# liusongxiang/efficient_tts

Hardware: AMD Instinct MI355X
Metric: mel-frames/sec (EFTS-CNN forward, batch 64/GPU, 80-mel LJSpeech shape) (higher is better)
Workload: dtype bf16; 1 GPU; EFTS-CNN forward (teacher-forced, no_grad) B=64 phon=128 mel=800 80-bin; batch_per_gpu=64, phoneme_len=128, mel_len=800, precision=bf16, parallelism=replicas x1

## Files before the change

### efficient_tts_amd/csrc/efts_prenet.hip

```cpp
#include <hip/hip_runtime.h>
#include <stdint.h>

#include "efts_rowsweep.h"

namespace efts {

struct FlArgs {
    const float* x;
    const char* w;
    const float* bias;
    float* y_f32;
    char* y;
    char* y_lo;
    long ldw, ldo, ldy;
    int B, T, Tp, cin, n;
    int act;
    float slope;
    int y_split;
};

constexpr int FL_NCB = 4;

template <int SPLIT, int KS>
__global__ __launch_bounds__(512, 2) void frame_linear_kernel(FlArgs p) {
    extern __shared__ __attribute__((aligned(16))) char smem[];
    constexpr int WF_BYTES = KS * FL_NCB * SPLIT * 1024;
    const int tid = threadIdx.x, lane = tid & 63, wave = tid >> 6, lrow = lane & 31, lhalf = lane >> 5;
    const int ncq = p.n / (32 * FL_NCB);
    const int ns = (p.cin + 15) >> 4;
    for (int unit = blockIdx.x; unit < p.B * ncq; unit += gridDim.x) {
    const int b = unit / ncq, cq = unit - b * ncq;
    const int c0 = cq * 32 * FL_NCB;
    if (unit != (int)blockIdx.x) __syncthreads();

    for (int idx = tid; idx < ns * FL_NCB * 64; idx += 512) {
        const int l = idx & 63, cb = (idx >> 6) % FL_NCB, s = idx / (64 * FL_NCB);
        const int k0 = 16 * s + 8 * (l >> 5);
        const char* src = p.w + (long)(c0 + cb * 32 + (l & 31)) * p.ldw + (SPLIT == 1 ? k0 * 2 : (k0 >> 5) * 128 + (k0 & 31) * 2);
        char* d = smem + ((s * FL_NCB + cb) * SPLIT) * 1024 + l * 16;
        *(u32x4*)d = *(const u32x4*)src;
        if constexpr (SPLIT == 2) *(u32x4*)(d + 1024) = *(const u32x4*)(src + 64);
    }
    float bv[FL_NCB];
#pragma unroll
    for (int cb = 0; cb < FL_NCB; ++cb) bv[cb] = p.bias ? p.bias[c0 + cb * 32 + lrow] : 0.f;
    __syncthreads();

    char* const st = smem + WF_BYTES + wave * 8192;
    const RowOut o{p.y_f32, p.y, p.y_lo, p.ldo, p.ldy, p.y_split};
    const int nrb = (p.T + 31) >> 5;
    for (int rb = wave; rb < nrb; rb += 8) {
        const int t = rb * 32 + lrow;
        const bool live = t < p.T;
        const float* xr = p.x + ((long)b * p.T + (live ? t : 0)) * p.cin;
        bf16x8 ah[KS], al[SPLIT == 2 ? KS : 1];
        (void)al;
#pragma unroll
        for (int s = 0; s < KS; ++s) {
            const int k0 = s * 16 + lhalf * 8;
            float f[8];
#pragma unroll
            for (int u = 0; u < 8; ++u) f[u] = 0.f;
            if (live && s < ns && k0 + 8 <= p.cin) {
                const float4 q0 = *(const float4*)(xr + k0), q1 = *(const float4*)(xr + k0 + 4);
                f[0] = q0.x; f[1] = q0.y; f[2] = q0.z; f[3] = q0.w; f[4] = q1.x; f[5] = q1.y; f[6] = q1.z; f[7] = q1.w;
            }
            u32x4 h4, l4;
            split8(f, &h4, &l4);
            ah[s] = __builtin_bit_cast(bf16x8, h4);
            if constexpr (SPLIT == 2) al[s] = __builtin_bit_cast(bf16x8, l4);
        }
        f32x16 acc[FL_NCB];
#pragma unroll
        for (int cb = 0; cb < FL_NCB; ++cb)
#pragma unroll
            for (int r = 0; r < 16; ++r) acc[cb][r] = 0.f;
#pragma unroll
        for (int s = 0; s < KS; ++s) {
            if (s < ns) {
                bf16x8 bh[FL_NCB], bl[SPLIT == 2 ? FL_NCB : 1];
                (void)bl;
#pragma unroll
                for (int cb = 0; cb < FL_NCB; ++cb) {
                    const char* src = smem + ((s * FL_NCB + cb) * SPLIT) * 1024 + lane * 16;
                    bh[cb] = *(const bf16x8*)src;
                    if constexpr (SPLIT == 2) bl[cb] = *(const bf16x8*)(src + 1024);
                }
                if constexpr (SPLIT == 2) {
#pragma unroll
                    for (int cb = 0; cb < FL_NCB; ++cb) acc[cb] = __builtin_amdgcn_mfma_f32_32x32x16_bf16(al[s], bh[cb], acc[cb], 0, 0, 0);
#pragma unroll
                    for (int cb = 0; cb < FL_NCB; ++cb) acc[cb] = __builtin_amdgcn_mfma_f32_32x32x16_bf16(ah[s], bl[cb], acc[cb], 0, 0, 0);
                }
#pragma unroll
                for (int cb = 0; cb < FL_NCB; ++cb) acc[cb] = __builtin_amdgcn_mfma_f32_32x32x16_bf16(ah[s], bh[cb], acc[cb], 0, 0, 0);
            }
        }
#pragma unroll
        for (int hp = 0; hp < FL_NCB / 2; ++hp)
            sweep64<true>(acc[2 * hp], acc[2 * hp + 1], st, lane, o, (long)b * p.Tp + rb * 32, p.T - rb * 32, c0 + hp * 64, bv[2 * hp], bv[2 * hp + 1],
                          p.act, p.slope);
    }
    }
}

}

using namespace efts;

extern "C" int efts_frame_linear(const efts_frame_linear_args* a, void* stream) {
    if (!a) return efts_fail(EFTS_EINVAL, "efts_frame_linear: null args");
    if (!a->x || !a->w || (!a->y && !a->y_f32)) return efts_fail(EFTS_EINVAL, "efts_frame_linear: null operand / no output");
    if (!(a->split == 1 || a->split == 2) || (a->y && !(a->y_split == 1 || a->y_split == 2))) return efts_fail(EFTS_EINVAL, "efts_frame_linear: split / y_split must be 1 or 2");
    if (a->B <= 0 || a->T <= 0 || a->Tp < a->T || a->cin <= 0 || a->cin > 128 || (a->cin & 7) || a->n <= 0 || a->n % (32 * FL_NCB))
        return efts_fail(EFTS_ESHAPE, "efts_frame_linear: cin must be a multiple of 8 up to 128, n a multiple of 128, T <= Tp");
    const int kch = a->split == 1 ? 64 : 32, nchunk = (a->cin + kch - 1) / kch;
    if (a->ldw < (int64_t)nchunk * 128 || (a->ldw & 15) || ((uintptr_t)a->w & 15) || ((uintptr_t)a->x & 15) || ((a->cin * 4) & 15))
        return efts_fail(EFTS_EALIGN, "efts_frame_linear: weight plane stride / alignment, frames must be 16-byte aligned rows");
    if ((a->y && ((a->ldy & 15) || ((uintptr_t)a->y & 15) || ((uintptr_t)a->y_lo & 15))) || (a->y_f32 && ((a->ldo & 3) || ((uintptr_t)a->y_f32 & 15))))
        return efts_fail(EFTS_EALIGN, "efts_frame_linear: output rows must be 16-byte aligned");
    if (a->y_split == 2 && a->y_lo) return efts_fail(EFTS_EINVAL, "efts_frame_linear: y_lo is for split-1 output planes");
    FlArgs k;
    k.x = a->x; k.w = (const char*)a->w; k.bias = a->bias; k.y_f32 = a->y_f32; k.y = (char*)a->y; k.y_lo = (char*)a->y_lo;
    k.ldw = a->ldw; k.ldo = a->ldo; k.ldy = a->ldy; k.B = a->B; k.T = a->T; k.Tp = a->Tp; k.cin = a->cin; k.n = a->n;
    k.act = a->act; k.slope = a->slope; k.y_split = a->y ? a->y_split : 0;
    int wgs = a->B * (a->n / (32 * FL_NCB));
    if (a->max_workgroups > 0 && a->max_workgroups < wgs) wgs = a->max_workgroups;
    const dim3 grid((unsigned)wgs);
#define EFTS_FL(S, N)                                                                                                                \
    do {                                                                                                                             \
        static bool attr = false;                                                                                                    \
        if (!attr) { (void)hipFuncSetAttribute((const void*)frame_linear_kernel<S, N>, hipFuncAttributeMaxDynamicSharedMemorySize, 160 * 1024); attr = true; } \
        hipLaunchKernelGGL((frame_linear_kernel<S, N>), grid, dim3(512), (size_t)N * FL_NCB * S * 1024 + 8 * 8192, (hipStream_t)stream, k);  \
    } while (0)
    const bool small = a->cin <= 80;
    if (a->split == 1) { if (small) EFTS_FL(1, 5); else EFTS_FL(1, 8); }
    else { if (small) EFTS_FL(2, 5); else EFTS_FL(2, 8); }
#undef EFTS_FL
    return efts_check_launch("efts_frame_linear");
}
```

### efficient_tts_amd/csrc/efts_rowsweep.h

```cpp
#pragma once
#include "efts_mma.h"

namespace efts {

struct RowOut {
    float* y_f32;
    char* y;
    char* y_lo;
    long ldo, ldy;
    int y_split;
};

__device__ __forceinline__ void gstore_b128(void* p, u32x4 v) {
    *(u32x4*)p = v;
    asm volatile("s_nop 4" ::"v"(v));
}

__device__ __forceinline__ void split8(const float* f, u32x4* hi, u32x4* lo) {
    float r[8], d0, d1;
    *hi = u32x4{pack_bf16x2(f[0], f[1], &r[0], &r[1]), pack_bf16x2(f[2], f[3], &r[2], &r[3]),
                pack_bf16x2(f[4], f[5], &r[4], &r[5]), pack_bf16x2(f[6], f[7], &r[6], &r[7])};
    *lo = u32x4{pack_bf16x2(r[0], r[1], &d0, &d1), pack_bf16x2(r[2], r[3], &d0, &d1),
                pack_bf16x2(r[4], r[5], &d0, &d1), pack_bf16x2(r[6], r[7], &d0, &d1)};
}

template <bool EPI>
__device__ __forceinline__ void sweep64(const f32x16& a0, const f32x16& a1, char* st, int lane, const RowOut& o, long orow0,
                                        int rows_live, int col0, float b0, float b1, int act, float slope) {
    const int lrow = lane & 31, lhalf = lane >> 5;
#pragma unroll
    for (int jj = 0; jj < 2; ++jj)
#pragma unroll
        for (int r = 0; r < 16; ++r) {
            const int rl = (r & 3) + 8 * (r >> 2) + 4 * lhalf, col = jj * 32 + lrow;
            float v = jj ? a1[r] : a0[r];
            if (EPI) {
                v += jj ? b1 : b0;
                if (act == EFTS_ACT_LEAKY) v = v > 0.f ? v : v * slope;
                else if (act == EFTS_ACT_RELU) v = v > 0.f ? v : 0.f;
            }
            *(float*)(st + rl * 256 + (((col >> 2) ^ ((rl >> 1) & 1)) << 4) + (col & 3) * 4) = v;
        }
#pragma unroll
    for (int pass = 0; pass < 4; ++pass) {
        const int row = pass * 8 + (lane >> 3), c8 = lane & 7, sw = (row >> 1) & 1;
        const long orow = orow0 + row;
        const bool keep = row < rows_live;
        if (o.y_f32 || (o.y && o.y_split == 1)) {
            const float4 d0 = *(const float4*)(st + row * 256 + (((2 * c8) ^ sw) << 4));
            const float4 d1 = *(const float4*)(st + row * 256 + (((2 * c8 + 1) ^ sw) << 4));
            const int col = col0 + c8 * 8;
            if (keep) {
                if (o.y_f32) {
                    gstore_b128(o.y_f32 + orow * o.ldo + col, __builtin_bit_cast(u32x4, d0));
                    gstore_b128(o.y_f32 + orow * o.ldo + col + 4, __builtin_bit_cast(u32x4, d1));
                }
                if (o.y && o.y_split == 1) {
                    const float f[8] = {d0.x, d0.y, d0.z, d0.w, d1.x, d1.y, d1.z, d1.w};
                    u32x4 hi, lo;
                    split8(f, &hi, &lo);
                    gstore_b128(o.y + orow * o.ldy + (long)col * 2, hi);
                    if (o.y_lo) gstore_b128(o.y_lo + orow * o.ldy + (long)col * 2, lo);
                }
            }
        }
        if (o.y && o.y_split == 2) {
#pragma unroll
            for (int ch = 0; ch < 2; ++ch) {
                const int s0 = ch * 8 + 2 * (c8 & 3);
                const float4 d0 = *(const float4*)(st + row * 256 + ((s0 ^ sw) << 4));
                const float4 d1 = *(const float4*)(st + row * 256 + (((s0 + 1) ^ sw) << 4));
                const float f[8] = {d0.x, d0.y, d0.z, d0.w, d1.x, d1.y, d1.z, d1.w};
                u32x4 hi, lo;
                split8(f, &hi, &lo);
                if (keep) gstore_b128(o.y + orow * o.ldy + (long)((col0 >> 5) + ch) * 128 + c8 * 16, c8 < 4 ? hi : lo);
            }
        }
    }
}

}
```

Measured before the change: 33.78 million mel-frames/s.

## Split tail row blocks across wave pairs and halve sweep staging LDS

The frame-linear kernel now splits leftover row blocks (when fewer than half of the eight waves would have work) into two half-width column tasks, so pairs of waves share each tail block instead of one wave handling it alone. The output sweep stages 16 rows at a time, which cuts per-wave LDS staging from 8KB to 4KB. A-operand fragments are now converted inside the k-loop rather than kept resident across all k-steps, which lowers register pressure. The cost is more kernel code, extra template instances, and duplicated x loads for half-width tail blocks.

```diff
diff --git a/efficient_tts_amd/csrc/efts_prenet.hip b/efficient_tts_amd/csrc/efts_prenet.hip
--- a/efficient_tts_amd/csrc/efts_prenet.hip
+++ b/efficient_tts_amd/csrc/efts_prenet.hip
@@ -21,11 +21,64 @@
 
 constexpr int FL_NCB = 4;
 
+template <int SPLIT, int KS, int NC>
+__device__ __forceinline__ void fl_block(const FlArgs& p, const char* wf, char* st, const RowOut& o, int b, int rb, int cb0, int c0, int ns,
+                                         float bv0, float bv1, float bv2, float bv3, int lane) {
+    const int lrow = lane & 31, lhalf = lane >> 5;
+    const int t = rb * 32 + lrow;
+    const bool live = t < p.T;
+    const float* xr = p.x + ((long)b * p.T + (live ? t : 0)) * p.cin;
+    f32x16 acc[NC];
+#pragma unroll
+    for (int cb = 0; cb < NC; ++cb)
+#pragma unroll
+        for (int r = 0; r < 16; ++r) acc[cb][r] = 0.f;
+#pragma unroll
+    for (int s = 0; s < KS; ++s) {
+        if (s < ns) {
+            const int k0 = s * 16 + lhalf * 8;
+            float f[8];
+#pragma unroll
+            for (int u = 0; u < 8; ++u) f[u] = 0.f;
+            if (live && k0 + 8 <= p.cin) {
+                const float4 q0 = *(const float4*)(xr + k0), q1 = *(const float4*)(xr + k0 + 4);
+                f[0] = q0.x; f[1] = q0.y; f[2] = q0.z; f[3] = q0.w; f[4] = q1.x; f[5] = q1.y; f[6] = q1.z; f[7] = q1.w;
+            }
+            u32x4 h4, l4;
+            split8(f, &h4, &l4);
+            const bf16x8 ah = __builtin_bit_cast(bf16x8, h4), al = __builtin_bit_cast(bf16x8, l4);
+            (void)al;
+            bf16x8 bh[NC], bl[SPLIT == 2 ? NC : 1];
+            (void)bl;
+#pragma unroll
+            for (int cb = 0; cb < NC; ++cb) {
+                const char* src = wf + ((s * FL_NCB + cb0 + cb) * SPLIT) * 1024 + lane * 16;
+                bh[cb] = *(const bf16x8*)src;
+                if constexpr (SPLIT == 2) bl[cb] = *(const bf16x8*)(src + 1024);
+            }
+            if constexpr (SPLIT == 2) {
+#pragma unroll
+                for (int cb = 0; cb < NC; ++cb) acc[cb] = __builtin_amdgcn_mfma_f32_32x32x16_bf16(al, bh[cb], acc[cb], 0, 0, 0);
+#pragma unroll
+                for (int cb = 0; cb < NC; ++cb) acc[cb] = __builtin_amdgcn_mfma_f32_32x32x16_bf16(ah, bl[cb], acc[cb], 0, 0, 0);
+            }
+#pragma unroll
+            for (int cb = 0; cb < NC; ++cb) acc[cb] = __builtin_amdgcn_mfma_f32_32x32x16_bf16(ah, bh[cb], acc[cb], 0, 0, 0);
+        }
+    }
+#pragma unroll
+    for (int hp = 0; hp < NC / 2; ++hp) {
+        const bool up = NC == 2 ? cb0 != 0 : hp != 0;
+        sweep64_rows16<true>(acc[2 * hp], acc[2 * hp + 1], st, lane, o, (long)b * p.Tp + rb * 32, p.T - rb * 32, c0 + (cb0 + 2 * hp) * 32,
+                      up ? bv2 : bv0, up ? bv3 : bv1, p.act, p.slope);
+    }
+}
+
 template <int SPLIT, int KS>
 __global__ __launch_bounds__(512, 2) void frame_linear_kernel(FlArgs p) {
     extern __shared__ __attribute__((aligned(16))) char smem[];
     constexpr int WF_BYTES = KS * FL_NCB * SPLIT * 1024;
-    const int tid = threadIdx.x, lane = tid & 63, wave = tid >> 6, lrow = lane & 31, lhalf = lane >> 5;
+    const int tid = threadIdx.x, lane = tid & 63, wave = tid >> 6, lrow = lane & 31;
     const int ncq = p.n / (32 * FL_NCB);
     const int ns = (p.cin + 15) >> 4;
     for (int unit = blockIdx.x; unit < p.B * ncq; unit += gridDim.x) {
@@ -46,61 +99,12 @@
     for (int cb = 0; cb < FL_NCB; ++cb) bv[cb] = p.bias ? p.bias[c0 + cb * 32 + lrow] : 0.f;
     __syncthreads();
 
-    char* const st = smem + WF_BYTES + wave * 8192;
+    char* const st = smem + WF_BYTES + wave * SWEEP16_BYTES;
     const RowOut o{p.y_f32, p.y, p.y_lo, p.ldo, p.ldy, p.y_split};
     const int nrb = (p.T + 31) >> 5;
-    for (int rb = wave; rb < nrb; rb += 8) {
-        const int t = rb * 32 + lrow;
-        const bool live = t < p.T;
-        const float* xr = p.x + ((long)b * p.T + (live ? t : 0)) * p.cin;
-        bf16x8 ah[KS], al[SPLIT == 2 ? KS : 1];
-        (void)al;
-#pragma unroll
-        for (int s = 0; s < KS; ++s) {
-            const int k0 = s * 16 + lhalf * 8;
-            float f[8];
-#pragma unroll
-            for (int u = 0; u < 8; ++u) f[u] = 0.f;
-            if (live && s < ns && k0 + 8 <= p.cin) {
-                const float4 q0 = *(const float4*)(xr + k0), q1 = *(const float4*)(xr + k0 + 4);
-                f[0] = q0.x; f[1] = q0.y; f[2] = q0.z; f[3] = q0.w; f[4] = q1.x; f[5] = q1.y; f[6] = q1.z; f[7] = q1.w;
-            }
-            u32x4 h4, l4;
-            split8(f, &h4, &l4);
-            ah[s] = __builtin_bit_cast(bf16x8, h4);
-            if constexpr (SPLIT == 2) al[s] = __builtin_bit_cast(bf16x8, l4);
-        }
-        f32x16 acc[FL_NCB];
-#pragma unroll
-        for (int cb = 0; cb < FL_NCB; ++cb)
-#pragma unroll
-            for (int r = 0; r < 16; ++r) acc[cb][r] = 0.f;
-#pragma unroll
-        for (int s = 0; s < KS; ++s) {
-            if (s < ns) {
-                bf16x8 bh[FL_NCB], bl[SPLIT == 2 ? FL_NCB : 1];
-                (void)bl;
-#pragma unroll
-                for (int cb = 0; cb < FL_NCB; ++cb) {
-                    const char* src = smem + ((s * FL_NCB + cb) * SPLIT) * 1024 + lane * 16;
-                    bh[cb] = *(const bf16x8*)src;
-                    if constexpr (SPLIT == 2) bl[cb] = *(const bf16x8*)(src + 1024);
-                }
-                if constexpr (SPLIT == 2) {
-#pragma unroll
-                    for (int cb = 0; cb < FL_NCB; ++cb) acc[cb] = __builtin_amdgcn_mfma_f32_32x32x16_bf16(al[s], bh[cb], acc[cb], 0, 0, 0);
-#pragma unroll
-                    for (int cb = 0; cb < FL_NCB; ++cb) acc[cb] = __builtin_amdgcn_mfma_f32_32x32x16_bf16(ah[s], bl[cb], acc[cb], 0, 0, 0);
-                }
-#pragma unroll
-                for (int cb = 0; cb < FL_NCB; ++cb) acc[cb] = __builtin_amdgcn_mfma_f32_32x32x16_bf16(ah[s], bh[cb], acc[cb], 0, 0, 0);
-            }
-        }
-#pragma unroll
-        for (int hp = 0; hp < FL_NCB / 2; ++hp)
-            sweep64<true>(acc[2 * hp], acc[2 * hp + 1], st, lane, o, (long)b * p.Tp + rb * 32, p.T - rb * 32, c0 + hp * 64, bv[2 * hp], bv[2 * hp + 1],
-                          p.act, p.slope);
-    }
+    const int nwhole = (nrb & 7) >= 1 && (nrb & 7) <= 4 ? (nrb & ~7) : nrb;
+    for (int rb = wave; rb < nwhole; rb += 8) fl_block<SPLIT, KS, FL_NCB>(p, smem, st, o, b, rb, 0, c0, ns, bv[0], bv[1], bv[2], bv[3], lane);
+    if (wave < 2 * (nrb - nwhole)) fl_block<SPLIT, KS, FL_NCB / 2>(p, smem, st, o, b, nwhole + (wave >> 1), (wave & 1) * 2, c0, ns, bv[0], bv[1], bv[2], bv[3], lane);
     }
 }
 
@@ -131,7 +135,7 @@
     do {                                                                                                                             \
         static bool attr = false;                                                                                                    \
         if (!attr) { (void)hipFuncSetAttribute((const void*)frame_linear_kernel<S, N>, hipFuncAttributeMaxDynamicSharedMemorySize, 160 * 1024); attr = true; } \
-        hipLaunchKernelGGL((frame_linear_kernel<S, N>), grid, dim3(512), (size_t)N * FL_NCB * S * 1024 + 8 * 8192, (hipStream_t)stream, k);  \
+        hipLaunchKernelGGL((frame_linear_kernel<S, N>), grid, dim3(512), (size_t)N * FL_NCB * S * 1024 + 8 * SWEEP16_BYTES, (hipStream_t)stream, k);  \
     } while (0)
     const bool small = a->cin <= 80;
     if (a->split == 1) { if (small) EFTS_FL(1, 5); else EFTS_FL(1, 8); }
diff --git a/efficient_tts_amd/csrc/efts_rowsweep.h b/efficient_tts_amd/csrc/efts_rowsweep.h
--- a/efficient_tts_amd/csrc/efts_rowsweep.h
+++ b/efficient_tts_amd/csrc/efts_rowsweep.h
@@ -79,4 +79,64 @@
     }
 }
 
+constexpr int SWEEP16_BYTES = 4096;
+
+template <bool EPI>
+__device__ __forceinline__ void sweep64_rows16(const f32x16& a0, const f32x16& a1, char* st, int lane, const RowOut& o, long orow0,
+                                        int rows_live, int col0, float b0, float b1, int act, float slope) {
+    const int lrow = lane & 31, lhalf = lane >> 5;
+#pragma unroll
+    for (int h = 0; h < 2; ++h) {
+#pragma unroll
+        for (int jj = 0; jj < 2; ++jj)
+#pragma unroll
+            for (int r = 0; r < 8; ++r) {
+                const int rl = (r & 3) + 8 * (r >> 2) + 4 * lhalf, col = jj * 32 + lrow;
+                float v = jj ? a1[8 * h + r] : a0[8 * h + r];
+                if (EPI) {
+                    v += jj ? b1 : b0;
+                    if (act == EFTS_ACT_LEAKY) v = v > 0.f ? v : v * slope;
+                    else if (act == EFTS_ACT_RELU) v = v > 0.f ? v : 0.f;
+                }
+                *(float*)(st + rl * 256 + (((col >> 2) ^ ((rl >> 1) & 1)) << 4) + (col & 3) * 4) = v;
+            }
+#pragma unroll
+        for (int pass = 0; pass < 2; ++pass) {
+            const int rl = pass * 8 + (lane >> 3), row = 16 * h + rl, c8 = lane & 7, sw = (rl >> 1) & 1;
+            const long orow = orow0 + row;
+            const bool keep = row < rows_live;
+            if (o.y_f32 || (o.y && o.y_split == 1)) {
+                const float4 d0 = *(const float4*)(st + rl * 256 + (((2 * c8) ^ sw) << 4));
+                const float4 d1 = *(const float4*)(st + rl * 256 + (((2 * c8 + 1) ^ sw) << 4));
+                const int col = col0 + c8 * 8;
+                if (keep) {
+                    if (o.y_f32) {
+                        gstore_b128(o.y_f32 + orow * o.ldo + col, __builtin_bit_cast(u32x4, d0));
+                        gstore_b128(o.y_f32 + orow * o.ldo + col + 4, __builtin_bit_cast(u32x4, d1));
+                    }
+                    if (o.y && o.y_split == 1) {
+                        const float f[8] = {d0.x, d0.y, d0.z, d0.w, d1.x, d1.y, d1.z, d1.w};
+                        u32x4 hi, lo;
+                        split8(f, &hi, &lo);
+                        gstore_b128(o.y + orow * o.ldy + (long)col * 2, hi);
+                        if (o.y_lo) gstore_b128(o.y_lo + orow * o.ldy + (long)col * 2, lo);
+                    }
+                }
+            }
+            if (o.y && o.y_split == 2) {
+#pragma unroll
+                for (int ch = 0; ch < 2; ++ch) {
+                    const int s0 = ch * 8 + 2 * (c8 & 3);
+                    const float4 d0 = *(const float4*)(st + rl * 256 + ((s0 ^ sw) << 4));
+                    const float4 d1 = *(const float4*)(st + rl * 256 + (((s0 + 1) ^ sw) << 4));
+                    const float f[8] = {d0.x, d0.y, d0.z, d0.w, d1.x, d1.y, d1.z, d1.w};
+                    u32x4 hi, lo;
+                    split8(f, &hi, &lo);
+                    if (keep) gstore_b128(o.y + orow * o.ldy + (long)((col0 >> 5) + ch) * 128 + c8 * 16, c8 < 4 ? hi : lo);
+                }
+            }
+        }
+    }
 }
+
+}
```

After: 33.85 million mel-frames/s, median of 6. Within noise of the previous version (+0.2%).
